# mj-will/aspire

Measured on AMD Instinct MI355X. Metric: particle-steps/sec (N x n_steps), 1M particles d=32; log-evidence err vs ref, higher is better.
Workload: dtype f64

## Files before the change

aspire_amd/csrc/asmc_common.h:

```cpp
#pragma once
#include <hip/hip_runtime.h>
#include <stdint.h>
#include <stdio.h>
#include <string.h>

#include "../../include/asmc.h"

#define ASMC_WAVE 64
#define ASMC_BLOCK 256
#define ASMC_MAX_BLOCKS 2048
#define ASMC_SCAN_TILE 2048
#define ASMC_PCN_MAX_GRID (1 << 20)
#define ASMC_GAMMA_BATCH 8
#define ASMC_MAX_PCN_STEPS 2048
#define BM_SC_N 256
#define BM_LG_N 128
#define BM_TAB_N (BM_SC_N + BM_LG_N)

void asmc_set_error(const char* fmt, ...);
void asmc_bm_table_host(double* tab);
struct asmc_ctx;
int asmc_count_nonfinite_enqueue(asmc_ctx* ctx, int64_t n, const double* v, hipStream_t st);
unsigned long long* asmc_count_slot(asmc_ctx* ctx);
struct asmc_ctx;
void asmc_prof_begin(asmc_ctx* ctx, const char* label, const void* kernel, hipStream_t st);
void asmc_poison_lds(asmc_ctx* ctx, hipStream_t st);
void asmc_prof_end(asmc_ctx* ctx, hipStream_t st);
#define ASMC_PROF_MAX 8192
#define ASMC_PROF_VARIANTS 256
#define ASMC_FIRST_ARG_(a, ...) a
#define ASMC_LAUNCH(ctx, st, label, ...)   \
    do {                                   \
        (ctx)->rec_n = 0;  \
        (ctx)->cs_n = 0;   \
        if ((ctx)->poison_lds) asmc_poison_lds((ctx), (st)); \
        asmc_prof_begin((ctx), (label), reinterpret_cast<const void*>(ASMC_FIRST_ARG_(__VA_ARGS__, 0)), (st)); \
        hipLaunchKernelGGL(__VA_ARGS__);   \
        asmc_prof_end((ctx), (st));        \
    } while (0)

#define ASMC_HIP(call)                                                                      \
    do {                                                                                    \
        hipError_t _e = (call);                                                             \
        if (_e != hipSuccess) {                                                             \
            asmc_set_error("%s failed: %s (%s:%d)", #call, hipGetErrorString(_e), __FILE__, \
                           __LINE__);                                                       \
            return ASMC_ERR_HIP;                                                            \
        }                                                                                   \
    } while (0)

// ... 38 lines not shown
    double* d_rec;
    const void* rec_src[3];
    int64_t rec_n;
    unsigned count_gen;
    uint64_t rec_token;
    const void* rec_hold_src[3];
    int64_t rec_hold_n;
    uint64_t rec_hold_token;
    const void* cs_x;
    int64_t cs_n;
    int cs_d, cs_grid;
    void* d_ysoa;
    void* d_xpad;
    size_t xpad_bytes;
    int d_max_pad;
    double* d_student;
    double* h_student;
    size_t ysoa_bytes;
    long long* d_counts;
    double* d_rho;
    unsigned long long* d_stretch;
    unsigned long long* d_mh;
    unsigned int* d_tilectr;
    unsigned int* d_bar;
    unsigned int bar_base[17];
    unsigned long long flow_nonfinite;
    int poison_lds;
    int isw_disabled;
    unsigned long long* d_pcgtab;
    long long* d_select;
    unsigned long long ptab_tag, ysplit_seq;
    double* d_ptab;
    double* d_bmtab;
    double* d_mmtab;
    double* d_f16tab;
    size_t f16tab_bytes;
    int (*count_hook)(void*, asmc_stream);
    void* count_hook_user;
    long long* count_cell;
    int count_cells;
    int64_t count_n_global;
    int mutate_defer, mutate_pending_steps;
    hipEvent_t ev_mutate;
    hipEvent_t ev_is;
    int is_result_pending;
    unsigned long long lq_nan;
    void* rccl_allreduce;
    void* rccl_comm;
    void* rccl_allgather;
    double* shard_st;
    int64_t n_tiles_max;
    int gram_blocks;
    size_t gram_cap;
    unsigned long long pcg_inc[2];
    int pcg_tab_valid;
    int prof_on;
    int prof_n;
    hipEvent_t* prof_ev;
    const char** prof_label;
    int prof_nv;
    const void* prof_vfn[ASMC_PROF_VARIANTS];
    long long prof_vcnt[ASMC_PROF_VARIANTS];
    double* h_pinned;
    unsigned ref_status_gen;
    double* h_gram;
    double* d_ref;
// ... 65 lines not shown
```

aspire_amd/csrc/asmc_ctx.hip:

```cpp
#include <dlfcn.h>
#include <stdarg.h>

#include <math.h>

#include "asmc_common.h"

static thread_local char g_err[512] = "";

void asmc_set_error(const char* fmt, ...) {
    va_list ap;
    va_start(ap, fmt);
    vsnprintf(g_err, sizeof(g_err), fmt, ap);
    va_end(ap);
}

__global__ __launch_bounds__(256) void k_poison_lds(int words) {
    extern __shared__ unsigned int s_poison[];
    for (int i = threadIdx.x; i < words; i += 256) s_poison[i] = 0xFFFFFFFFu;
    __syncthreads();
    if (s_poison[(threadIdx.x * 977) % words] != 0xFFFFFFFFu) __builtin_trap();
}
void asmc_poison_lds(asmc_ctx* ctx, hipStream_t st) {
    const int bytes = 160 * 1024 - 1024;
    static bool attr_set_dev[ASMC_MAX_DEVICES] = {false}; bool& attr_set = attr_set_dev[asmc_dev_slot(ctx)];
// ... 151 lines not shown
        if (e == hipSuccess) e = hipMalloc(p, bytes);
    };
    dmalloc((void**)&c->d_partials, sizeof(double) * ASMC_MAX_BLOCKS * ASMC_MAX_BETAS * 2);
    dmalloc((void**)&c->d_small, sizeof(double) * 4096);
    dmalloc((void**)&c->d_keys, sizeof(unsigned long long) * (ASMC_MAX_BETAS + 8));
    dmalloc((void**)&c->d_tiles, sizeof(double) * (size_t)(c->n_tiles_max * 4 + 64));
    dmalloc((void**)&c->d_tiles_i, sizeof(long long) * (size_t)(c->n_tiles_max * 8 + 64));
    c->gram_cap = (size_t)c->gram_blocks * d_max * d_max;
    if (c->gram_cap < (size_t)2048 * 1024) c->gram_cap = (size_t)2048 * 1024;
    dmalloc((void**)&c->d_gram, sizeof(double) * c->gram_cap);
    c->d_mmtab = nullptr;
    c->poison_lds = getenv("ASMC_POISON_LDS") != nullptr;
    c->d_max_pad = d_max <= 4 ? 4 : d_max <= 8 ? 8 : d_max <= 16 ? 16 : d_max <= 32 ? 32 : d_max <= 64 ? 64 : d_max <= 128 ? 128 : 0;
    dmalloc((void**)&c->d_mmtab, sizeof(double) * 2 * 144 * 64);
    dmalloc((void**)&c->d_guide, sizeof(unsigned int) * ((size_t)n_max + 8));
    dmalloc((void**)&c->d_tilectr, ASMC_TILECTR_BYTES + (size_t)n_max + 64);
    c->d_flags = c->d_tilectr ? reinterpret_cast<unsigned char*>(c->d_tilectr) + ASMC_TILECTR_BYTES : nullptr;
    dmalloc((void**)&c->d_gamma, sizeof(double) * ((size_t)ASMC_GAMMA_BATCH * (size_t)n_max + 64 * ASMC_GAMMA_BATCH));
    dmalloc((void**)&c->d_rec, sizeof(double) * 4 * (size_t)n_max);
    const size_t student = (size_t)d_max * (d_max + 1) + (size_t)(ASMC_STUDENT_MAX_ROWS / 64) * (d_max + 2);
    dmalloc((void**)&c->d_student, sizeof(double) * student);
    if (e == hipSuccess) e = hipHostMalloc((void**)&c->h_student, sizeof(double) * student, hipHostMallocDefault);
    dmalloc((void**)&c->d_counts, sizeof(long long) * (size_t)(ASMC_MAX_PCN_STEPS + ASMC_MAX_BLOCKS + n_max / 64 + 8));
    dmalloc((void**)&c->d_rho, sizeof(double) * (ASMC_MAX_PCN_STEPS + 8));
    dmalloc((void**)&c->d_stretch, sizeof(unsigned long long) * ASMC_MAX_PCN_STEPS);
    dmalloc((void**)&c->d_mh, sizeof(unsigned long long) * ASMC_MAX_PCN_STEPS);
    if (e == hipSuccess) e = hipMemset(c->d_tilectr, 0, ASMC_TILECTR_BYTES);
    dmalloc((void**)&c->d_bar, sizeof(unsigned int) * 1024 * 17);
    if (e == hipSuccess) e = hipMemset(c->d_bar, 0, sizeof(unsigned int) * 1024 * 17);
    dmalloc((void**)&c->d_pcgtab, sizeof(unsigned long long) * (64 * 4 + 8));
    dmalloc((void**)&c->d_select, sizeof(long long) * (2 * (ASMC_SELECT_THREADS / 64) + 8));
    dmalloc((void**)&c->d_ptab, sizeof(double) * (2 * 32 * 32 + 32 + 3 * ASMC_MAX_COMPONENTS * (1 + 2 * 32) + 64));
    dmalloc((void**)&c->d_bmtab, sizeof(double) * 2 * BM_TAB_N);
    dmalloc((void**)&c->d_ref, sizeof(double) * (128 + 128 * 128));
    if (e == hipSuccess) {
        double tab[2 * BM_TAB_N];
        asmc_bm_table_host(tab);
        e = hipMemcpy(c->d_bmtab, tab, sizeof(tab), hipMemcpyHostToDevice);
    }
    if (e == hipSuccess) e = hipHostMalloc((void**)&c->h_pinned, sizeof(double) * 8192, hipHostMallocDefault);
    if (e == hipSuccess) e = hipHostMalloc((void**)&c->h_gram, sizeof(double) * (128 + 128 * 128), hipHostMallocDefault);
    if (e != hipSuccess) {
        asmc_set_error("asmc_ctx_create: allocation failed: %s", hipGetErrorString(e));
        asmc_ctx_destroy(c);
        return ASMC_ERR_NOMEM;
    }
    *ctx_out = c;
    return ASMC_OK;
}

int asmc_ctx_destroy(asmc_ctx* c) {
    if (!c) return ASMC_OK;
    (void)hipSetDevice(c->device);
    (void)hipFree(c->d_partials);
    (void)hipFree(c->d_small);
    (void)hipFree(c->d_keys);
    (void)hipFree(c->d_tiles);
    (void)hipFree(c->d_tiles_i);
    (void)hipFree(c->d_gram);
    if (c->d_mmtab) (void)hipFree(c->d_mmtab);
    if (c->d_f16tab) (void)hipFree(c->d_f16tab);
    (void)hipFree(c->d_guide);
    (void)hipFree(c->d_gamma);
    (void)hipFree(c->d_student);
    if (c->h_student) (void)hipHostFree(c->h_student);
    if (c->d_ysoa) (void)hipFree(c->d_ysoa);
    if (c->d_xpad) (void)hipFree(c->d_xpad);
    (void)hipFree(c->d_counts);
    (void)hipFree(c->d_rho);
    (void)hipFree(c->d_stretch);
    (void)hipFree(c->d_mh);
    (void)hipFree(c->d_tilectr);
    (void)hipFree(c->d_rec);
    (void)hipFree(c->d_bar);
    (void)hipFree(c->d_pcgtab);
    (void)hipFree(c->d_select);
    (void)hipFree(c->d_ptab);
    (void)hipFree(c->d_bmtab);
    (void)hipFree(c->d_ref);
    if (c->prof_ev) {
        for (int i = 0; i < 2 * ASMC_PROF_MAX; i++) (void)hipEventDestroy(c->prof_ev[i]);
        delete[] c->prof_ev;
        delete[] c->prof_label;
    }
    if (c->h_pinned) (void)hipHostFree(c->h_pinned);
    if (c->h_gram) (void)hipHostFree(c->h_gram);
    if (c->ev_mutate) (void)hipEventDestroy(c->ev_mutate);
    if (c->ev_is) (void)hipEventDestroy(c->ev_is);
    delete c;
    return ASMC_OK;
}

}
```

aspire_amd/csrc/asmc_flow_dev.h:

```cpp
#pragma once
#include "asmc_common.h"

typedef float floatx16 __attribute__((ext_vector_type(16)));


__device__ __forceinline__ float flow_standardise(float x, float loc, float scale, float rcp) {
    const float a = x - loc;
    const float q0 = a * rcp;
    const float r = fmaf(-scale, q0, a);
    return fmaf(r, rcp, q0);
}

typedef float flow_std2 __attribute__((ext_vector_type(2)));
__device__ __forceinline__ flow_std2 flow_standardise2(flow_std2 x, flow_std2 loc, flow_std2 scale, flow_std2 rcp) {
    const flow_std2 a = x - loc;
    const flow_std2 q0 = a * rcp;
    const flow_std2 r = __builtin_elementwise_fma(-scale, q0, a);
    return __builtin_elementwise_fma(r, rcp, q0);
}

template <bool INVERSE>
__device__ __forceinline__ void flow_affine(float& x, float sraw, float t, float& ladj, int form) {
    if (form == 0) {
        const float sv = 2.0f - 4.0f * __builtin_amdgcn_rcpf(__expf(sraw) + 1.0f);
// ... 579 lines not shown
            if (overlap) {
#pragma unroll
                for (int c = 0; c < 4; c++)
                    if (c * NM / 4 == m) cvt(g + 1, c, c == 3);
            }
            __builtin_amdgcn_sched_barrier(0);
        }
        if (more) {
            if (!overlap) {
#pragma unroll
                for (int c = 0; c < 4; c++) cvt(g + 1, c, c == 3);
            }
            bh = pack(hp), bl = pack(lq);
            if (PREFETCH) {
#pragma unroll
                for (int nb = 0; nb < NBM; nb++) ah[nb] = ahn[nb], al[nb] = aln[nb];
            } else {
                a_load(g + 1, ah, al);
            }
            __builtin_amdgcn_sched_barrier(0);
        }
    }
    flow_f2 lacc = {0.0f, 0.0f};
#pragma unroll
    for (int q = 0; q < H / 2; q += 2)
        flow_affine2<false>(trans[q], trans[q + 1], o[q / 16][q % 16], o[(q + 1) / 16][(q + 1) % 16], o[(H / 2 + q) / 16][(H / 2 + q) % 16],
                            o[(H / 2 + q + 1) / 16][(H / 2 + q + 1) % 16], lacc, FORM >= 0 ? FORM : form);
    ladj += lacc.x + lacc.y;
}

template <int H, int W, int THREADS>
__device__ __forceinline__ void flow_stage_hs(float* __restrict__ sp, const float* __restrict__ packed, int n_layers) {
    using FD = FlowDims<H, W>;
    constexpr int L4 = FD::LAYER / 4, B4 = FD::BIAS / 4;
    const int total4 = n_layers * L4;
    for (int i4 = threadIdx.x; i4 < total4; i4 += THREADS) {
        const int in_layer = i4 % L4;
        if (in_layer < B4) {
            reinterpret_cast<float4*>(sp)[i4] = reinterpret_cast<const float4*>(packed)[i4];
            continue;
        }
        const int local = in_layer - B4;
        if ((local / 64) & 1) continue;
        const float4 f0 = reinterpret_cast<const float4*>(packed)[i4], f1 = reinterpret_cast<const float4*>(packed)[i4 + 64];
        const float xv[8] = {f0.x, f0.y, f0.z, f0.w, f1.x, f1.y, f1.z, f1.w};
        half8 hi, lo;
        float wmax = 0.0f;
        split8_f16<false>(xv, hi, lo, wmax);
        reinterpret_cast<half8*>(sp)[i4] = hi;
        reinterpret_cast<half8*>(sp)[i4 + 64] = lo;
    }
}
```

aspire_amd/csrc/asmc_pcn.hip:

```cpp
#include <stdlib.h>

#include <chrono>

#include "asmc_common.h"
#include "asmc_tile.h"
#include "asmc_pcn_dev.h"
#include "asmc_transform_dev.h"

template <typename T>
__device__ __forceinline__ double mixture_eval(const MixDev& m, int d, const char* row) {
    double best = -INFINITY;
    double terms[ASMC_MAX_COMPONENTS];
    const int C = m.C;
    for (int c = 0; c < C; c++) {
        double q = 0.0;
        const double* mu = m.mu + (size_t)c * d;
        const double* pr = m.prec + (size_t)c * d;
        for (int j = 0; j < d; j++) {
            const double t = row_get<T>(row, j) - mu[j];
            q = fma(t * t, pr[j], q);
        }
        const double v = m.logw[c] - 0.5 * q;
        terms[c] = v;
        best = fmax(best, v);
// ... 2911 lines not shown
        ASMC_LAUNCH_CHECK();
    }
    if (reg_ok) {
        pd.beta = prm->beta;
        pd.ll = to_dev(prm->log_likelihood);
        pd.lp = to_dev(prm->log_prior);
        pd.lq = pd.lp;
        pd.noise = prm->noise;
        ASMC_REQUIRE(pd.noise == ASMC_NOISE_F64 || pd.noise == ASMC_NOISE_F32, "bad noise mode");
        rc = pack_pcn_tables(ctx, pd, st, d_rho, *rho_inout_host);
        if (rc) return rc;
        long long* d_block = ctx->d_counts + ASMC_MAX_PCN_STEPS;
        int grid = 0;
        const bool soa = pcn_ensure_ysoa(ctx, n, d, prm->x_dtype, pd, st, asmc_pcn_flow_fused_ok(prm, flow));
        auto convert = [&](int mode) -> int {
            PcnDev pc = pd;
            pc.mode = !soa ? mode : mode == PCN_WHITEN ? PCN_WHITEN_S : PCN_UNWHITEN_XS;
            pc.noise = ASMC_NOISE_F64;
            if (prm->x_dtype == ASMC_F64)
                return launch_pcn_step<double, 0>(ctx, n, (double*)x, ll, lp, lq, pc, d_rho, 0, d_block, &grid, nullptr, nullptr, nullptr, st);
            return launch_pcn_step<float, 0>(ctx, n, (float*)x, ll, lp, lq, pc, d_rho, 0, d_block, &grid, nullptr, nullptr, nullptr, st);
        };
        rc = convert(PCN_WHITEN);
        if (rc) return rc;
        const bool fused = soa && asmc_pcn_flow_fused_ok(prm, flow);
        if (d_noise > 0 && !fused) {
            asmc_set_error("asmc_pcn_mutate_flow: the zero-padded form needs the one-kernel step");
            return ASMC_ERR_UNSUPPORTED;
        }
        if (fused) {
            ASMC_HIP(hipMemsetAsync(ctx->d_tilectr, 0, ASMC_TILECTR_BYTES + ((size_t)((n + 63) / 64) + 15) / 16 * 16, st));
            pd.tile_par = ctx->d_flags;
        }
        for (int t = 0; t < (fused ? n_steps : 0); t++) {
            const uint32_t step = step0 + (uint32_t)t;
            rc = pcn_prepare_gamma(ctx, n, pd, step, st);
            if (rc) return rc;
            PcnAdaptArgs ad = {ctx->d_tilectr + ASMC_MAX_PCN_STEPS + t,
                               reinterpret_cast<unsigned long long*>(ctx->d_tilectr + 2 * ASMC_MAX_PCN_STEPS),
                               ctx->count_hook ? ctx->count_cell : nullptr,
                               ctx->count_hook && t > 0 ? ctx->count_cell : nullptr, d_counts, d_rho, d_rho_hist,
                               prm->target_accept, ctx->count_hook ? ctx->count_n_global : n, t, prm->adapt, t == n_steps - 1};
            const int lag = prm->adapt >= 2 ? prm->adapt : 1;
            if (ctx->count_hook && lag > ctx->count_cells) {
                asmc_set_error("adapt_lag %d needs %d exchange cells, the installed hook has %d (asmc_pcn_set_count_cells)", lag, lag, ctx->count_cells);
                return ASMC_ERR_ARG;
            }
            rc = asmc_pcn_flow_fused_launch(ctx, n, prm->x_dtype == ASMC_F64 ? ASMC_F64 : ASMC_F32, ll, lp, lq, pd, flow, d_rho, step,
                                            ctx->d_tilectr + t, d_block, &grid, ad, st);
            if (rc) return rc;
            if (ctx->count_hook && ((t + 1) % lag == 0 || t == n_steps - 1)) {
                const int hrc = ctx->count_hook(ctx->count_hook_user, reinterpret_cast<asmc_stream>(st));
                if (hrc != 0) {
                    asmc_set_error("accept-count exchange hook failed (%d)", hrc);
                    return ASMC_ERR_ARG;
                }
                if (t == n_steps - 1) {
                    ASMC_LAUNCH(ctx, st, "k_pcn_adapt", k_pcn_adapt, dim3(1), dim3(1024), 0, st, 1,
                                (const long long*)ctx->count_cell, ctx->count_n_global, t, d_counts, d_rho, d_rho_hist,
                                prm->target_accept, prm->adapt, (const double*)(d_rho_hist + t), 1,
                                lag > 1 ? (const long long*)ctx->count_cell : (const long long*)nullptr);
                    ASMC_LAUNCH_CHECK();
                }
            }
        }
        for (int t = 0; t < (fused ? 0 : n_steps); t++) {
            const uint32_t step = step0 + (uint32_t)t;
            rc = pcn_prepare_gamma(ctx, n, pd, step, st);
            if (rc) return rc;
#define FLOW_STEP(TT, MD)                                                                                               \
    dispatch_pcn_reg_flow<TT, MD>(ctx, n, (TT*)x, (TT*)x_prop, ll, lp, lq, ll_new, lp_new, lq_new, pd, d_rho, step, d_block, \
                                  &grid, st)
            if (prm->x_dtype == ASMC_F64)
                rc = soa ? FLOW_STEP(double, PCN_FLOW_PROPOSE_S) : FLOW_STEP(double, PCN_FLOW_PROPOSE);
            else
                rc = soa ? FLOW_STEP(float, PCN_FLOW_PROPOSE_S) : FLOW_STEP(float, PCN_FLOW_PROPOSE);
            if (rc) return rc;
            rc = asmc_coupling_logprob(ctx, n, prm->x_dtype, x_prop, flow, lq_new, stream);
            if (rc) return rc;
            if (prm->x_dtype == ASMC_F64)
                rc = soa ? FLOW_STEP(double, PCN_FLOW_ACCEPT_S) : FLOW_STEP(double, PCN_FLOW_ACCEPT);
            else
// ... 309 lines not shown
```

aspire_amd/csrc/asmc_pcn_dev.h:

```cpp
#pragma once
#include "asmc_common.h"

bool asmc_flow_math_split();

struct PcnAdaptArgs {
    unsigned int* done;
    unsigned long long* nonfinite;
    long long* cell;
    const long long* prev_cell;
    long long* counts_out;
    double* rho;
    double* rho_hist;
    double target;
    int64_t n;
    int t, adapt;
    int last;
};

__device__ __forceinline__ double pcn_adapt_rho(double rho, long long c, int64_t n, double target, int t) {
    const double acc = (double)c / (double)n;
    double r = exp(log(rho) + (acc - target) / pow((double)(t + 1), 0.75));
    r = r < 1e-4 ? 1e-4 : r;
    r = r > 0.99 ? 0.99 : r;
    return r;
// ... 328 lines not shown
    int d_real;
    unsigned long long seed, gid0;
    int c_ll, c_lp, c_lq;
    const double* bmtab;
    unsigned char* tile_par;
    int d_noise;
};


template <typename T>
__device__ __forceinline__ double soa_load(__amdgpu_buffer_rsrc_t r, unsigned voff, unsigned soff) {
    if constexpr (sizeof(T) == 8) {
        const auto v = __builtin_amdgcn_raw_buffer_load_b64(r, (int)voff, (int)soff, 0);
        return __builtin_bit_cast(double, v);
    } else {
        const unsigned v = __builtin_amdgcn_raw_buffer_load_b32(r, (int)voff, (int)soff, 0);
        return (double)__uint_as_float(v);
    }
}
template <typename T>
__device__ __forceinline__ void soa_store(__amdgpu_buffer_rsrc_t r, unsigned voff, unsigned soff, double x) {
    if constexpr (sizeof(T) == 8) {
        using u2 = decltype(__builtin_amdgcn_raw_buffer_load_b64(r, 0, 0, 0));
        __builtin_amdgcn_raw_buffer_store_b64(__builtin_bit_cast(u2, x), r, (int)voff, (int)soff, 0);
    } else {
        __builtin_amdgcn_raw_buffer_store_b32(__float_as_uint((float)x), r, (int)voff, (int)soff, 0);
    }
}


bool asmc_pcn_flow_fused_ok(const asmc_pcn_params* prm, const asmc_coupling* f);
int asmc_pcn_flow_fused_launch(asmc_ctx* ctx, int64_t n, int x_dtype, double* ll, double* lp, double* lq, const PcnDev& pd,
                               const asmc_coupling* f, const double* rho_ptr, uint32_t step, unsigned int* tile_counter,
                               long long* block_counts, int* grid_out, const PcnAdaptArgs& adapt, hipStream_t st);

#define MM_WHITEN 0
#define MM_STEP 1
#define MM_UNWHITEN 2
#define MM_STEP_T 3
#define MM_XPROPOSE 4
#define MM_XPROPOSE_T 5
#define MM_UNWHITEN_X 6
bool asmc_pcn_mm_supported(int d, const void* x);
int asmc_pcn_mm_pack(asmc_ctx* ctx, const PcnDev& pd, hipStream_t st);
int asmc_pcn_flow16_tables(asmc_ctx* ctx, const PcnDev& pd, const asmc_coupling* f, hipStream_t st);
int asmc_pcn_flow16_launch(asmc_ctx* ctx, int64_t n, int x_dtype, void* x, double* ll, double* lp, double* lq, const PcnDev& pd,
                           const asmc_coupling* f, const double* rho_ptr, uint32_t step, long long* block_counts, int* grid_out,
                           unsigned long long* nonfinite, hipStream_t st);
int asmc_pcn_mm_launch(asmc_ctx* ctx, int64_t n, int x_dtype, void* x, double* ll, double* lp, double* lq, const PcnDev& pd,
                       int mode, const double* rho_ptr, uint32_t step, long long* block_counts, int* grid_out,
                       hipStream_t st);
bool asmc_gram_mm_supported(int d, const void* x);
int asmc_gram_mm_launch(asmc_ctx* ctx, int64_t n, int d, int x_dtype, const void* x, const double* d_center, int* grid_out,
                        hipStream_t st, double* out2, double n_div);
```

aspire_amd/csrc/asmc_pcn_fused.hip:

```cpp
#include <stdlib.h>

#include "asmc_common.h"
#include <type_traits>
#include "asmc_pcn_dev.h"
#include "asmc_flow_dev.h"

#ifndef FUSED_THREADS
#define FUSED_THREADS 512
#endif

#define FUSED_TL_DOUBLES 1368
#define FUSED_MAX_COMPONENTS 4
#ifndef MV_DEPTH
#define MV_DEPTH 4
#endif
typedef double double2v __attribute__((ext_vector_type(2)));
__host__ __device__ constexpr int mv_group(int bi) {
    int g = 0;
    while ((g + 1) * (g + 2) <= bi) g++;
    return g;
}
template <int I, int N, typename F>
__device__ __forceinline__ void mv_for_each(F& f) {
    if constexpr (I < N) {
        f(std::integral_constant<int, I>{});
        mv_for_each<I + 1, N>(f);
    }
}
#ifndef FUSED_INPLACE
#define FUSED_INPLACE 1
#endif
#ifndef FUSED_MVMFMA
#define FUSED_MVMFMA FUSED_INPLACE
#endif
typedef double fused_d4 __attribute__((ext_vector_type(4)));
__device__ __forceinline__ void fused_swap32(double& x, double& y) {
    const unsigned long long xb = __builtin_bit_cast(unsigned long long, x), yb = __builtin_bit_cast(unsigned long long, y);
    const auto lo = __builtin_amdgcn_permlane32_swap((unsigned)xb, (unsigned)yb, false, false);
    const auto hi = __builtin_amdgcn_permlane32_swap((unsigned)(xb >> 32), (unsigned)(yb >> 32), false, false);
    x = __builtin_bit_cast(double, ((unsigned long long)hi[0] << 32) | lo[0]);
    y = __builtin_bit_cast(double, ((unsigned long long)hi[1] << 32) | lo[1]);
}
__device__ __forceinline__ void fused_swap16(double& x, double& y) {
    const unsigned long long xb = __builtin_bit_cast(unsigned long long, x), yb = __builtin_bit_cast(unsigned long long, y);
    const auto lo = __builtin_amdgcn_permlane16_swap((unsigned)xb, (unsigned)yb, false, false);
    const auto hi = __builtin_amdgcn_permlane16_swap((unsigned)(xb >> 32), (unsigned)(yb >> 32), false, false);
    x = __builtin_bit_cast(double, ((unsigned long long)hi[0] << 32) | lo[0]);
    y = __builtin_bit_cast(double, ((unsigned long long)hi[1] << 32) | lo[1]);
}
__device__ __forceinline__ void fused_transpose4(double& q0, double& q1, double& q2, double& q3) {
    fused_swap32(q0, q2);
    fused_swap32(q1, q3);
    fused_swap16(q0, q1);
    fused_swap16(q2, q3);
}
#ifndef HS1P_PREFETCH
#define HS1P_PREFETCH false
#endif
#ifndef FUSED_PRIO_A
#define FUSED_PRIO_A 2
#define FUSED_PRIO_B 1
#endif
#ifndef MV_CHUNK
#define MV_CHUNK 8
#endif
template <typename T, int W, int NOISE, bool HS, int KIND = ASMC_FLOW_COUPLING, bool MIX = false>
__global__ __launch_bounds__(FUSED_THREADS) void k_pcn_flow_fused(
    int64_t n, double* __restrict__ ll, double* __restrict__ lp, double* __restrict__ lq, const double* __restrict__ ptab,
    PcnScalars p, const double* rho_ptr, uint32_t step, const float* __restrict__ packed, int n_layers,
    const float* __restrict__ loc, const float* __restrict__ scale, float ladj0, float base_const,
    unsigned int* __restrict__ tile_counter, long long* __restrict__ block_counts, PcnAdaptArgs ad, int par_words, int affine) {
    constexpr int D = 32, H = 16, THREADS = FUSED_THREADS;
    constexpr int HF = KIND == ASMC_FLOW_MAF ? 32 : H;
    static_assert(KIND == ASMC_FLOW_COUPLING || HS, "the autoregressive variant runs the split-fp16 layers only");
    using FD = FlowDims<HF, W>;
    extern __shared__ __align__(16) float sp[];
    if (HS) {
        flow_stage_hs<HF, W, THREADS>(sp, packed, n_layers);
    } else {
        const int total4 = n_layers * FD::LAYER / 4;
        for (int base = 0; base < total4; base += THREADS * 8) {
            float4 tmp[8];
#pragma unroll
            for (int q = 0; q < 8; q++) {
                const int i4 = base + q * THREADS + threadIdx.x;
                tmp[q] = i4 < total4 ? reinterpret_cast<const float4*>(packed)[i4] : make_float4(0.f, 0.f, 0.f, 0.f);
            }
#pragma unroll
            for (int q = 0; q < 8; q++) {
                const int i4 = base + q * THREADS + threadIdx.x;
                if (i4 < total4) reinterpret_cast<float4*>(sp)[i4] = tmp[q];
            }
        }
    }
    double* tl = reinterpret_cast<double*>(sp + (size_t)n_layers * FD::LAYER);
    constexpr int T_MU = D * D, T_LLMU = T_MU + D, T_LLPR = T_LLMU + D, T_LPMU = T_LLPR + D, T_LPPR = T_LPMU + D,
                  T_LOGW = T_LPPR + D, T_LOC = T_LOGW + 2;
    static_assert(T_LOC + 3 * D / 2 <= FUSED_TL_DOUBLES, "pCN tables");
    constexpr int M_MU = 12 * 64, M_MIX = M_MU + D, M_LOGW = M_MIX + 2 * FUSED_MAX_COMPONENTS * 2 * D, M_LOC = M_LOGW + 2 * FUSED_MAX_COMPONENTS;
    static_assert(M_LOC + 3 * D / 2 <= FUSED_TL_DOUBLES, "pCN tables (matrix-core variant)");
    constexpr bool MVM = FUSED_MVMFMA && FUSED_INPLACE;
    {
        const double* m0g = ptab + 2 * PTAB_TRI(D) + D;
        const int dr = (p.d_noise > 0 && p.d_noise < D) ? p.d_noise : D;
        const int dhalf = KIND == ASMC_FLOW_MAF ? 16 : dr / 2;
        auto nat = [&](int r) -> int {
            const int c = r < 16 ? (r < dhalf ? r : -1) : (r - 16 + dhalf);
            return (c >= 0 && c < dr) ? c : -1;
        };
        if (MVM) {
            for (int e = threadIdx.x; e < 12 * 64; e += THREADS) {
                const int slot = e >> 6, l = e & 63, mb = slot < 4 ? 0 : 1, sidx = slot < 4 ? slot : slot - 4;
                const int i = l & 15, j = nat(16 * mb + 4 * (i & 3) + (i >> 2)), k = 4 * sidx + (l >> 4);
                tl[e] = (j >= 0 && k <= j) ? ptab[j * (j + 1) / 2 + k] : 0.0;
            }
            for (int e = threadIdx.x; e < D; e += THREADS) {
                const int j = nat(16 * ((e >> 2) & 1) + 4 * (e >> 3) + (e & 3));
                tl[M_MU + e] = j >= 0 ? ptab[2 * PTAB_TRI(D) + j] : 0.0;
                reinterpret_cast<float*>(tl + M_LOC)[e] = j >= 0 ? loc[j] : 0.0f;
                reinterpret_cast<float*>(tl + M_LOC)[D + e] = j >= 0 ? scale[j] : 1.0f;
                reinterpret_cast<float*>(tl + M_LOC)[2 * D + e] = j >= 0 ? 1.0f / scale[j] : 1.0f;
            }
            for (int e = threadIdx.x; e < 2 * FUSED_MAX_COMPONENTS * D; e += THREADS) {
                const int tc = e / D, er = e % D, tt = tc / FUSED_MAX_COMPONENTS, c = tc % FUSED_MAX_COMPONENTS;
                const int j = nat(16 * ((er >> 2) & 1) + 4 * (er >> 3) + (er & 3));
                const bool live = j >= 0 && c < (tt == 0 ? p.c_ll : p.c_lp);
                const double* mg = m0g + (size_t)tt * PTAB_MIX(D);
                tl[M_MIX + tc * 2 * D + er] = live ? mg[ASMC_MAX_COMPONENTS + c * D + j] : 0.0;
                tl[M_MIX + tc * 2 * D + D + er] = live ? mg[ASMC_MAX_COMPONENTS * (1 + D) + c * D + j] : 0.0;
            }
            if (threadIdx.x < 2 * FUSED_MAX_COMPONENTS) {
                const int tt = threadIdx.x / FUSED_MAX_COMPONENTS, c = threadIdx.x % FUSED_MAX_COMPONENTS;
                tl[M_LOGW + threadIdx.x] = c < (tt == 0 ? p.c_ll : p.c_lp) ? m0g[(size_t)tt * PTAB_MIX(D) + c] : -INFINITY;
            }
        } else {
            for (int e = threadIdx.x; e < D * D; e += THREADS) {
                const int j = e / D, k = e - j * D;
                tl[e] = k <= j ? ptab[j * (j + 1) / 2 + k] : 0.0;
            }
            for (int e = threadIdx.x; e < D; e += THREADS) {
                tl[T_MU + e] = ptab[2 * PTAB_TRI(D) + e];
                tl[T_LLMU + e] = m0g[ASMC_MAX_COMPONENTS + e];
                tl[T_LLPR + e] = m0g[ASMC_MAX_COMPONENTS * (1 + D) + e];
                tl[T_LPMU + e] = m0g[PTAB_MIX(D) + ASMC_MAX_COMPONENTS + e];
                tl[T_LPPR + e] = m0g[PTAB_MIX(D) + ASMC_MAX_COMPONENTS * (1 + D) + e];
                reinterpret_cast<float*>(tl + T_LOC)[e] = loc[e];
                reinterpret_cast<float*>(tl + T_LOC)[D + e] = scale[e];
                reinterpret_cast<float*>(tl + T_LOC)[2 * D + e] = 1.0f / scale[e];
            }
        }
        if (!MVM && threadIdx.x == 0) tl[T_LOGW] = m0g[0], tl[T_LOGW + 1] = m0g[PTAB_MIX(D)];
    }
    bm_d2* bmt = reinterpret_cast<bm_d2*>(tl + FUSED_TL_DOUBLES);
    if (NOISE == ASMC_NOISE_F64) bm_tab_stage<THREADS>(bmt, p.bmtab);
    unsigned* const par_bits = reinterpret_cast<unsigned*>(bmt + BM_TAB_N);
    for (int wd = threadIdx.x; wd < par_words; wd += THREADS) {
        const uint4 b0 = reinterpret_cast<const uint4*>(p.tile_par)[2 * wd], b1 = reinterpret_cast<const uint4*>(p.tile_par)[2 * wd + 1];
        const unsigned q[8] = {b0.x, b0.y, b0.z, b0.w, b1.x, b1.y, b1.z, b1.w};
        unsigned bits = 0;
#pragma unroll
        for (int k = 0; k < 8; k++) {
            const unsigned nib = (((q[k] & 0x01010101u) * 0x01020408u) >> 24) & 0xFu;
            bits |= nib << (4 * k);
        }
        par_bits[wd] = bits;
    }
    __syncthreads();
    const int lane = threadIdx.x & 63, wave = threadIdx.x >> 6, hh = lane >> 5;
    const bool first_on_simd = __builtin_amdgcn_readfirstlane(wave) < 4;
#ifdef FUSED_STAGGER
    if (!first_on_simd) {
#pragma unroll 1
        for (int i = 0; i < FUSED_STAGGER; i++) __builtin_amdgcn_s_sleep(127);
    }
#endif
    double rho;
    if (ad.prev_cell) {
        const double rp = ad.rho_hist[ad.t - 1];
        if (ad.adapt <= 1) {
            const long long cp = *ad.prev_cell;
            rho = ad.adapt ? pcn_adapt_rho(rp, cp, ad.n, ad.target, ad.t - 1) : rp;
            if (blockIdx.x == 0 && threadIdx.x == 0) ad.counts_out[ad.t - 1] = cp;
        } else if (ad.t % ad.adapt == 0) {
            double r = rp;
            for (int tp = ad.t - ad.adapt; tp < ad.t; tp++) {
                const long long ct = ad.prev_cell[tp % ad.adapt];
                r = pcn_adapt_rho(r, ct, ad.n, ad.target, tp);
                if (blockIdx.x == 0 && threadIdx.x == 0) ad.counts_out[tp] = ct;
            }
            rho = r;
        } else {
            rho = rp;
        }
    } else {
        rho = *rho_ptr;
    }
    if (ad.cell && blockIdx.x == 0 && threadIdx.x == 0) ad.rho_hist[ad.t] = rho;
    const double a = sqrt(1.0 - rho * rho);
// ... 609 lines not shown
        const unsigned int tk = __hip_atomic_fetch_add(ad.done, 1u, __ATOMIC_RELAXED, __HIP_MEMORY_SCOPE_AGENT);
        s_last = (tk == gridDim.x - 1u);
        if (s_last) __builtin_amdgcn_fence(__ATOMIC_ACQUIRE, "agent");
    }
    __syncthreads();
    if (!s_last) return;
    long long c = 0;
    for (int b = threadIdx.x; b < (int)gridDim.x; b += THREADS)
        c += __hip_atomic_load(&block_counts[b], __ATOMIC_RELAXED, __HIP_MEMORY_SCOPE_AGENT);
    c = wave_sum_ll(c);
    __syncthreads();
    if (lane == 0) s_cnt[wave] = c;
    __syncthreads();
    if (threadIdx.x == 0) {
        c = 0;
        for (int w = 0; w < THREADS / 64; w++) c += s_cnt[w];
        if (ad.cell) {
            ad.cell[ad.adapt >= 2 ? ad.t % ad.adapt : 0] = c;
            return;
        }
        ad.counts_out[ad.t] = c;
        ad.rho_hist[ad.t] = rho;
        if (ad.adapt == 1) {
            *ad.rho = pcn_adapt_rho(rho, c, ad.n, ad.target, ad.t);
        } else if (ad.adapt >= 2 && ((ad.t + 1) % ad.adapt == 0 || ad.last)) {
            double r = rho;
            for (int tp = ad.t - (ad.t % ad.adapt); tp <= ad.t; tp++)
                r = pcn_adapt_rho(r, tp == ad.t ? c : ad.counts_out[tp], ad.n, ad.target, tp);
            *ad.rho = r;
        }
    }
}

template <typename T>
static int launch_pcn_flow_fused(asmc_ctx* ctx, int64_t n, double* ll, double* lp, double* lq, const PcnDev& pd,
                                 const asmc_coupling* f, const double* rho_ptr, uint32_t step, unsigned int* tile_counter,
                                 long long* block_counts, int* grid_out, const PcnAdaptArgs& adapt, hipStream_t st) {
    PcnScalars ps;
    ps.beta = pd.beta;
    ps.nu = pd.nu;
    ps.gam = pd.gam;
    ps.ys = pd.ys;
    ps.n_pad = pd.n_pad;
    ps.d_real = pd.d;
    ps.d_noise = pd.d_noise;
    ps.seed = pd.seed;
    ps.gid0 = pd.gid0;
    ps.c_ll = pd.ll.C;
    ps.c_lp = pd.lp.C;
    ps.c_lq = 0;
    ps.bmtab = pd.bmtab;
    ps.tile_par = pd.tile_par;
    const float ladj0 = (float)(-f->log_scale_sum);
    const float base_const = (float)(-0.5 * f->dims * 1.8378770664093453);
    const int64_t n_tiles = (n + 63) / 64;
    const int grid = (int)(n_tiles < (int64_t)ctx->num_cu * (FUSED_THREADS / 64) ? (n_tiles + FUSED_THREADS / 64 - 1) / (FUSED_THREADS / 64) : ctx->num_cu);
    *grid_out = grid;
    const bool hs = asmc_flow_math_split();
    const bool mix = pd.ll.C > 1 || pd.lp.C > 1;
#define ASMC_FUSED_CASE_K(WW, NZ, HSV, KD) ASMC_FUSED_CASE_KM(WW, NZ, HSV, KD, false)
#define ASMC_FUSED_CASE_KM(WW, NZ, HSV, KD, MX)                                                                           \
    if (f->hidden == WW && pd.noise == NZ && hs == HSV && f->kind == KD && mix == MX) {                                   \
        auto kern = k_pcn_flow_fused<T, WW, NZ, HSV, KD, MX>;                                                                 \
        const size_t lds0 = (size_t)f->n_layers * FlowDims<(KD == ASMC_FLOW_MAF ? 32 : 16), WW>::LAYER * sizeof(float) + FUSED_TL_DOUBLES * sizeof(double) + BM_TAB_N * sizeof(bm_d2); \
        const size_t par_bytes = (size_t)((n_tiles + 31) / 32) * 4;    \
        const int par_words = (!FUSED_INPLACE && lds0 + par_bytes <= 160 * 1024) ? (int)(par_bytes / 4) : 0;                     \
        const size_t lds = lds0 + (size_t)par_words * 4;                                                                     \
        static size_t attr_lds_dev[ASMC_MAX_DEVICES] = {0}; size_t& attr_lds = attr_lds_dev[asmc_dev_slot(ctx)];                                                                                      \
        if (lds > 64 * 1024 && lds > attr_lds) {                                                                         \
            ASMC_HIP(hipFuncSetAttribute(reinterpret_cast<const void*>(kern), hipFuncAttributeMaxDynamicSharedMemorySize, (int)lds)); \
            attr_lds = lds;                                                                                              \
        }                                                                                                                \
        ASMC_LAUNCH(ctx, st, "k_pcn_flow_fused", kern, dim3(grid), dim3(FUSED_THREADS), lds, st, n, ll, lp, lq,                     \
                    (const double*)ctx->d_ptab, ps, rho_ptr, step, f->packed_dev, (int)f->n_layers, f->loc_dev, f->scale_dev, \
                    ladj0, base_const, tile_counter, block_counts, adapt, par_words, KD == ASMC_FLOW_MAF ? (int)f->affine : 0);  \
        ASMC_LAUNCH_CHECK();                                                                                             \
        return ASMC_OK;                                                                                                  \
    }
#define ASMC_FUSED_CASE(WW, NZ, HSV) ASMC_FUSED_CASE_K(WW, NZ, HSV, ASMC_FLOW_COUPLING)
    ASMC_FUSED_CASE(64, ASMC_NOISE_F64, true)
#ifndef FUSED_ONLY_HEADLINE
    ASMC_FUSED_CASE_KM(64, ASMC_NOISE_F64, true, ASMC_FLOW_COUPLING, true)
    ASMC_FUSED_CASE_KM(64, ASMC_NOISE_F32, true, ASMC_FLOW_COUPLING, true)
    ASMC_FUSED_CASE(64, ASMC_NOISE_F64, false)
    ASMC_FUSED_CASE(64, ASMC_NOISE_F32, true)
    ASMC_FUSED_CASE(64, ASMC_NOISE_F32, false)
    ASMC_FUSED_CASE(32, ASMC_NOISE_F64, true)
    ASMC_FUSED_CASE(32, ASMC_NOISE_F64, false)
    ASMC_FUSED_CASE(32, ASMC_NOISE_F32, true)
    ASMC_FUSED_CASE(32, ASMC_NOISE_F32, false)
    ASMC_FUSED_CASE(128, ASMC_NOISE_F64, true)
    ASMC_FUSED_CASE(128, ASMC_NOISE_F64, false)
    ASMC_FUSED_CASE(128, ASMC_NOISE_F32, true)
    ASMC_FUSED_CASE(128, ASMC_NOISE_F32, false)
    ASMC_FUSED_CASE_K(64, ASMC_NOISE_F64, true, ASMC_FLOW_MAF)
    ASMC_FUSED_CASE_K(64, ASMC_NOISE_F32, true, ASMC_FLOW_MAF)
    ASMC_FUSED_CASE_K(32, ASMC_NOISE_F64, true, ASMC_FLOW_MAF)
    ASMC_FUSED_CASE_K(32, ASMC_NOISE_F32, true, ASMC_FLOW_MAF)
#endif
#undef ASMC_FUSED_CASE
#undef ASMC_FUSED_CASE_K
#undef ASMC_FUSED_CASE_KM
    asmc_set_error("fused flow step: unsupported flow (kind %d, hidden width %d)", (int)f->kind, (int)f->hidden);
    return ASMC_ERR_UNSUPPORTED;
}

bool asmc_pcn_flow_fused_ok(const asmc_pcn_params* prm, const asmc_coupling* f) {
    if (getenv("ASMC_FLOW_SPLIT")) return false;
    if (prm->d != 32 || f->dims > 32 || f->dims < 2) return false;
    if (f->dims != 32 && !(FUSED_MVMFMA && FUSED_INPLACE)) return false;
    if (f->kind == ASMC_FLOW_COUPLING && (f->dims % 2)) return false;
    const bool mvm = FUSED_MVMFMA && FUSED_INPLACE && f->kind == ASMC_FLOW_COUPLING && f->hidden == 64 && asmc_flow_math_split();
    const int cmax = mvm ? FUSED_MAX_COMPONENTS : 1;
    if (prm->log_likelihood.n_components < 1 || prm->log_likelihood.n_components > cmax) return false;
    if (prm->log_prior.n_components < 1 || prm->log_prior.n_components > cmax) return false;
    if (!(f->hidden == 32 || f->hidden == 64 || f->hidden == 128)) return false;
    if (f->kind == ASMC_FLOW_MAF) {
        if (!asmc_flow_math_split() || f->hidden == 128) return false;
        const size_t per_tr = (size_t)((2 * (f->hidden / 32) + 2) * 32 + f->hidden * 32 + f->hidden * f->hidden + 2 * 32 * f->hidden) * sizeof(float);
        return per_tr * (size_t)f->n_layers + FUSED_TL_DOUBLES * sizeof(double) + BM_TAB_N * sizeof(bm_d2) <= 160 * 1024;
    }
    const size_t per_layer = (size_t)((2 * (f->hidden / 32) + 1) * 32 + f->hidden * 16 + f->hidden * f->hidden + 2 * 16 * f->hidden) * sizeof(float);
    return per_layer * (size_t)f->n_layers + FUSED_TL_DOUBLES * sizeof(double) + BM_TAB_N * sizeof(bm_d2) <= 160 * 1024;
}


int asmc_pcn_flow_fused_launch(asmc_ctx* ctx, int64_t n, int x_dtype, double* ll, double* lp, double* lq, const PcnDev& pd,
                               const asmc_coupling* f, const double* rho_ptr, uint32_t step, unsigned int* tile_counter,
                               long long* block_counts, int* grid_out, const PcnAdaptArgs& adapt, hipStream_t st) {
    if (x_dtype == ASMC_F64)
        return launch_pcn_flow_fused<double>(ctx, n, ll, lp, lq, pd, f, rho_ptr, step, tile_counter, block_counts, grid_out, adapt, st);
    return launch_pcn_flow_fused<float>(ctx, n, ll, lp, lq, pd, f, rho_ptr, step, tile_counter, block_counts, grid_out, adapt, st);
}
```

Baseline: 3.495 billion.

## Prebuild fused-kernel LDS image once per sweep and bulk-copy it per block

Adds a one-block staging kernel that builds the fused pCN step's LDS contents once per call: split-fp16 flow weights, pCN tables and the Box-Muller table, written to a device buffer. Each block of the per-step fused kernel then loads this image with wide coalesced reads held in registers and stores it to LDS, instead of recomputing the fp16 splits and tables itself. The inline staging loop is also batched so more global loads are in flight at once. The aim is to cut per-block prologue cost, at the price of many extra registers per thread to hold the image (up to 160 KB split over the block) and one extra launch per sweep. An environment variable can restore inline staging.

After: 3.553 billion (median of 6 runs). 1.7% higher.

```diff
diff --git a/aspire_amd/csrc/asmc_common.h b/aspire_amd/csrc/asmc_common.h
--- a/aspire_amd/csrc/asmc_common.h
+++ b/aspire_amd/csrc/asmc_common.h
@@ -16,6 +16,7 @@
 #define BM_SC_N 256
 #define BM_LG_N 128
 #define BM_TAB_N (BM_SC_N + BM_LG_N)
+#define ASMC_FUSED_IMAGE_BYTES (160 * 1024)
 
 void asmc_set_error(const char* fmt, ...);
 void asmc_bm_table_host(double* tab);
@@ -120,6 +121,7 @@
     unsigned long long ptab_tag, ysplit_seq;
     double* d_ptab;
     double* d_bmtab;
+    void* d_fimg;
     double* d_mmtab;
     double* d_f16tab;
     size_t f16tab_bytes;
diff --git a/aspire_amd/csrc/asmc_ctx.hip b/aspire_amd/csrc/asmc_ctx.hip
--- a/aspire_amd/csrc/asmc_ctx.hip
+++ b/aspire_amd/csrc/asmc_ctx.hip
@@ -207,6 +207,7 @@
     dmalloc((void**)&c->d_select, sizeof(long long) * (2 * (ASMC_SELECT_THREADS / 64) + 8));
     dmalloc((void**)&c->d_ptab, sizeof(double) * (2 * 32 * 32 + 32 + 3 * ASMC_MAX_COMPONENTS * (1 + 2 * 32) + 64));
     dmalloc((void**)&c->d_bmtab, sizeof(double) * 2 * BM_TAB_N);
+    dmalloc((void**)&c->d_fimg, ASMC_FUSED_IMAGE_BYTES);
     dmalloc((void**)&c->d_ref, sizeof(double) * (128 + 128 * 128));
     if (e == hipSuccess) {
         double tab[2 * BM_TAB_N];
@@ -252,6 +253,7 @@
     (void)hipFree(c->d_select);
     (void)hipFree(c->d_ptab);
     (void)hipFree(c->d_bmtab);
+    (void)hipFree(c->d_fimg);
     (void)hipFree(c->d_ref);
     if (c->prof_ev) {
         for (int i = 0; i < 2 * ASMC_PROF_MAX; i++) (void)hipEventDestroy(c->prof_ev[i]);
diff --git a/aspire_amd/csrc/asmc_flow_dev.h b/aspire_amd/csrc/asmc_flow_dev.h
--- a/aspire_amd/csrc/asmc_flow_dev.h
+++ b/aspire_amd/csrc/asmc_flow_dev.h
@@ -635,22 +635,35 @@
 template <int H, int W, int THREADS>
 __device__ __forceinline__ void flow_stage_hs(float* __restrict__ sp, const float* __restrict__ packed, int n_layers) {
     using FD = FlowDims<H, W>;
-    constexpr int L4 = FD::LAYER / 4, B4 = FD::BIAS / 4;
+    constexpr int L4 = FD::LAYER / 4, B4 = FD::BIAS / 4, BATCH = 8;
     const int total4 = n_layers * L4;
-    for (int i4 = threadIdx.x; i4 < total4; i4 += THREADS) {
-        const int in_layer = i4 % L4;
-        if (in_layer < B4) {
-            reinterpret_cast<float4*>(sp)[i4] = reinterpret_cast<const float4*>(packed)[i4];
-            continue;
-        }
-        const int local = in_layer - B4;
-        if ((local / 64) & 1) continue;
-        const float4 f0 = reinterpret_cast<const float4*>(packed)[i4], f1 = reinterpret_cast<const float4*>(packed)[i4 + 64];
-        const float xv[8] = {f0.x, f0.y, f0.z, f0.w, f1.x, f1.y, f1.z, f1.w};
-        half8 hi, lo;
-        float wmax = 0.0f;
-        split8_f16<false>(xv, hi, lo, wmax);
-        reinterpret_cast<half8*>(sp)[i4] = hi;
-        reinterpret_cast<half8*>(sp)[i4 + 64] = lo;
-    }
-}
+    const float4* __restrict__ g4 = reinterpret_cast<const float4*>(packed);
+    for (int base = threadIdx.x; base < total4; base += THREADS * BATCH) {
+        float4 f0[BATCH], f1[BATCH];
+#pragma unroll
+        for (int q = 0; q < BATCH; q++) {
+            const int i4 = base + q * THREADS, in_layer = i4 % L4;
+            const bool in = i4 < total4, bias = in_layer < B4;
+            const bool pair = in && !bias && !(((in_layer - B4) / 64) & 1);
+            f0[q] = f1[q] = make_float4(0.f, 0.f, 0.f, 0.f);
+            if ((in && bias) || pair) f0[q] = g4[i4];
+            if (pair) f1[q] = g4[i4 + 64];
+        }
+#pragma unroll
+        for (int q = 0; q < BATCH; q++) {
+            const int i4 = base + q * THREADS, in_layer = i4 % L4;
+            if (i4 >= total4) continue;
+            if (in_layer < B4) {
+                reinterpret_cast<float4*>(sp)[i4] = f0[q];
+                continue;
+            }
+            if (((in_layer - B4) / 64) & 1) continue;
+            const float xv[8] = {f0[q].x, f0[q].y, f0[q].z, f0[q].w, f1[q].x, f1[q].y, f1[q].z, f1[q].w};
+            half8 hi, lo;
+            float wmax = 0.0f;
+            split8_f16<false>(xv, hi, lo, wmax);
+            reinterpret_cast<half8*>(sp)[i4] = hi;
+            reinterpret_cast<half8*>(sp)[i4 + 64] = lo;
+        }
+    }
+}
diff --git a/aspire_amd/csrc/asmc_pcn.hip b/aspire_amd/csrc/asmc_pcn.hip
--- a/aspire_amd/csrc/asmc_pcn.hip
+++ b/aspire_amd/csrc/asmc_pcn.hip
@@ -2967,6 +2967,11 @@
             ASMC_HIP(hipMemsetAsync(ctx->d_tilectr, 0, ASMC_TILECTR_BYTES + ((size_t)((n + 63) / 64) + 15) / 16 * 16, st));
             pd.tile_par = ctx->d_flags;
         }
+        int img_words = 0;
+        if (fused) {
+            rc = asmc_pcn_flow_fused_stage(ctx, pd, flow, &img_words, st);
+            if (rc) return rc;
+        }
         for (int t = 0; t < (fused ? n_steps : 0); t++) {
             const uint32_t step = step0 + (uint32_t)t;
             rc = pcn_prepare_gamma(ctx, n, pd, step, st);
@@ -2982,7 +2987,7 @@
                 return ASMC_ERR_ARG;
             }
             rc = asmc_pcn_flow_fused_launch(ctx, n, prm->x_dtype == ASMC_F64 ? ASMC_F64 : ASMC_F32, ll, lp, lq, pd, flow, d_rho, step,
-                                            ctx->d_tilectr + t, d_block, &grid, ad, st);
+                                            ctx->d_tilectr + t, d_block, &grid, ad, img_words, st);
             if (rc) return rc;
             if (ctx->count_hook && ((t + 1) % lag == 0 || t == n_steps - 1)) {
                 const int hrc = ctx->count_hook(ctx->count_hook_user, reinterpret_cast<asmc_stream>(st));
diff --git a/aspire_amd/csrc/asmc_pcn_dev.h b/aspire_amd/csrc/asmc_pcn_dev.h
--- a/aspire_amd/csrc/asmc_pcn_dev.h
+++ b/aspire_amd/csrc/asmc_pcn_dev.h
@@ -384,7 +384,8 @@
 bool asmc_pcn_flow_fused_ok(const asmc_pcn_params* prm, const asmc_coupling* f);
 int asmc_pcn_flow_fused_launch(asmc_ctx* ctx, int64_t n, int x_dtype, double* ll, double* lp, double* lq, const PcnDev& pd,
                                const asmc_coupling* f, const double* rho_ptr, uint32_t step, unsigned int* tile_counter,
-                               long long* block_counts, int* grid_out, const PcnAdaptArgs& adapt, hipStream_t st);
+                               long long* block_counts, int* grid_out, const PcnAdaptArgs& adapt, int img_words, hipStream_t st);
+int asmc_pcn_flow_fused_stage(asmc_ctx* ctx, const PcnDev& pd, const asmc_coupling* f, int* words_out, hipStream_t st);
 
 #define MM_WHITEN 0
 #define MM_STEP 1
diff --git a/aspire_amd/csrc/asmc_pcn_fused.hip b/aspire_amd/csrc/asmc_pcn_fused.hip
--- a/aspire_amd/csrc/asmc_pcn_fused.hip
+++ b/aspire_amd/csrc/asmc_pcn_fused.hip
@@ -34,6 +34,7 @@
 #define FUSED_MVMFMA FUSED_INPLACE
 #endif
 typedef double fused_d4 __attribute__((ext_vector_type(4)));
+typedef unsigned fused_u4 __attribute__((ext_vector_type(4)));
 __device__ __forceinline__ void fused_swap32(double& x, double& y) {
     const unsigned long long xb = __builtin_bit_cast(unsigned long long, x), yb = __builtin_bit_cast(unsigned long long, y);
     const auto lo = __builtin_amdgcn_permlane32_swap((unsigned)xb, (unsigned)yb, false, false);
@@ -64,17 +65,20 @@
 #ifndef MV_CHUNK
 #define MV_CHUNK 8
 #endif
-template <typename T, int W, int NOISE, bool HS, int KIND = ASMC_FLOW_COUPLING, bool MIX = false>
-__global__ __launch_bounds__(FUSED_THREADS) void k_pcn_flow_fused(
-    int64_t n, double* __restrict__ ll, double* __restrict__ lp, double* __restrict__ lq, const double* __restrict__ ptab,
-    PcnScalars p, const double* rho_ptr, uint32_t step, const float* __restrict__ packed, int n_layers,
-    const float* __restrict__ loc, const float* __restrict__ scale, float ladj0, float base_const,
-    unsigned int* __restrict__ tile_counter, long long* __restrict__ block_counts, PcnAdaptArgs ad, int par_words, int affine) {
-    constexpr int D = 32, H = 16, THREADS = FUSED_THREADS;
-    constexpr int HF = KIND == ASMC_FLOW_MAF ? 32 : H;
-    static_assert(KIND == ASMC_FLOW_COUPLING || HS, "the autoregressive variant runs the split-fp16 layers only");
+constexpr int FUSED_D = 32;
+constexpr int T_MU = FUSED_D * FUSED_D, T_LLMU = T_MU + FUSED_D, T_LLPR = T_LLMU + FUSED_D, T_LPMU = T_LLPR + FUSED_D, T_LPPR = T_LPMU + FUSED_D,
+              T_LOGW = T_LPPR + FUSED_D, T_LOC = T_LOGW + 2;
+static_assert(T_LOC + 3 * FUSED_D / 2 <= FUSED_TL_DOUBLES, "pCN tables");
+constexpr int M_MU = 12 * 64, M_MIX = M_MU + FUSED_D, M_LOGW = M_MIX + 2 * FUSED_MAX_COMPONENTS * 2 * FUSED_D, M_LOC = M_LOGW + 2 * FUSED_MAX_COMPONENTS;
+static_assert(M_LOC + 3 * FUSED_D / 2 <= FUSED_TL_DOUBLES, "pCN tables (matrix-core variant)");
+constexpr bool MVM = FUSED_MVMFMA && FUSED_INPLACE;
+
+template <int W, int NOISE, bool HS, int KIND>
+__device__ __forceinline__ void fused_stage_tables(float* __restrict__ sp, const double* __restrict__ ptab, const PcnScalars& p,
+                                                   const float* __restrict__ packed, int n_layers, const float* __restrict__ loc,
+                                                   const float* __restrict__ scale) {
+    constexpr int D = FUSED_D, THREADS = FUSED_THREADS, HF = KIND == ASMC_FLOW_MAF ? 32 : 16;
     using FD = FlowDims<HF, W>;
-    extern __shared__ __align__(16) float sp[];
     if (HS) {
         flow_stage_hs<HF, W, THREADS>(sp, packed, n_layers);
     } else {
@@ -94,12 +98,6 @@
         }
     }
     double* tl = reinterpret_cast<double*>(sp + (size_t)n_layers * FD::LAYER);
-    constexpr int T_MU = D * D, T_LLMU = T_MU + D, T_LLPR = T_LLMU + D, T_LPMU = T_LLPR + D, T_LPPR = T_LPMU + D,
-                  T_LOGW = T_LPPR + D, T_LOC = T_LOGW + 2;
-    static_assert(T_LOC + 3 * D / 2 <= FUSED_TL_DOUBLES, "pCN tables");
-    constexpr int M_MU = 12 * 64, M_MIX = M_MU + D, M_LOGW = M_MIX + 2 * FUSED_MAX_COMPONENTS * 2 * D, M_LOC = M_LOGW + 2 * FUSED_MAX_COMPONENTS;
-    static_assert(M_LOC + 3 * D / 2 <= FUSED_TL_DOUBLES, "pCN tables (matrix-core variant)");
-    constexpr bool MVM = FUSED_MVMFMA && FUSED_INPLACE;
     {
         const double* m0g = ptab + 2 * PTAB_TRI(D) + D;
         const int dr = (p.d_noise > 0 && p.d_noise < D) ? p.d_noise : D;
@@ -151,8 +149,48 @@
         }
         if (!MVM && threadIdx.x == 0) tl[T_LOGW] = m0g[0], tl[T_LOGW + 1] = m0g[PTAB_MIX(D)];
     }
+    if (NOISE == ASMC_NOISE_F64) bm_tab_stage<THREADS>(reinterpret_cast<bm_d2*>(tl + FUSED_TL_DOUBLES), p.bmtab);
+}
+template <int W, int NOISE, int KIND>
+__host__ __device__ constexpr int fused_image_words(int n_layers) {
+    return (int)(((size_t)n_layers * FlowDims<(KIND == ASMC_FLOW_MAF ? 32 : 16), W>::LAYER * sizeof(float) + FUSED_TL_DOUBLES * sizeof(double) +
+                  (NOISE == ASMC_NOISE_F64 ? BM_TAB_N * sizeof(bm_d2) : 0)) / 16);
+}
+template <int W, int NOISE, bool HS, int KIND>
+__global__ __launch_bounds__(FUSED_THREADS) void k_fused_stage_image(const double* __restrict__ ptab, PcnScalars p, const float* __restrict__ packed,
+                                                                     int n_layers, const float* __restrict__ loc, const float* __restrict__ scale,
+                                                                     fused_u4* __restrict__ img, int img_words) {
+    extern __shared__ __align__(16) float sp[];
+    fused_stage_tables<W, NOISE, HS, KIND>(sp, ptab, p, packed, n_layers, loc, scale);
+    __syncthreads();
+    for (int i = threadIdx.x; i < img_words; i += FUSED_THREADS) img[i] = reinterpret_cast<const fused_u4*>(sp)[i];
+}
+
+template <typename T, int W, int NOISE, bool HS, int KIND = ASMC_FLOW_COUPLING, bool MIX = false>
+__global__ __launch_bounds__(FUSED_THREADS) void k_pcn_flow_fused(
+    int64_t n, double* __restrict__ ll, double* __restrict__ lp, double* __restrict__ lq, const double* __restrict__ ptab,
+    PcnScalars p, const double* rho_ptr, uint32_t step, const float* __restrict__ packed, int n_layers,
+    const float* __restrict__ loc, const float* __restrict__ scale, float ladj0, float base_const,
+    unsigned int* __restrict__ tile_counter, long long* __restrict__ block_counts, PcnAdaptArgs ad, int par_words, int affine,
+    const fused_u4* __restrict__ img, int img_words) {
+    constexpr int D = FUSED_D, H = 16, THREADS = FUSED_THREADS;
+    constexpr int HF = KIND == ASMC_FLOW_MAF ? 32 : H;
+    static_assert(KIND == ASMC_FLOW_COUPLING || HS, "the autoregressive variant runs the split-fp16 layers only");
+    using FD = FlowDims<HF, W>;
+    extern __shared__ __align__(16) float sp[];
+    constexpr int IMG_Q = ASMC_FUSED_IMAGE_BYTES / 16 / THREADS;
+    fused_u4 iw[IMG_Q];
+    if (img != nullptr) {
+#pragma unroll
+        for (int q = 0; q < IMG_Q; q++) {
+            const int i4 = q * THREADS + (int)threadIdx.x;
+            iw[q] = img[i4 < img_words ? i4 : img_words - 1];
+        }
+    } else {
+        fused_stage_tables<W, NOISE, HS, KIND>(sp, ptab, p, packed, n_layers, loc, scale);
+    }
+    double* tl = reinterpret_cast<double*>(sp + (size_t)n_layers * FD::LAYER);
     bm_d2* bmt = reinterpret_cast<bm_d2*>(tl + FUSED_TL_DOUBLES);
-    if (NOISE == ASMC_NOISE_F64) bm_tab_stage<THREADS>(bmt, p.bmtab);
     unsigned* const par_bits = reinterpret_cast<unsigned*>(bmt + BM_TAB_N);
     for (int wd = threadIdx.x; wd < par_words; wd += THREADS) {
         const uint4 b0 = reinterpret_cast<const uint4*>(p.tile_par)[2 * wd], b1 = reinterpret_cast<const uint4*>(p.tile_par)[2 * wd + 1];
@@ -164,6 +202,14 @@
             bits |= nib << (4 * k);
         }
         par_bits[wd] = bits;
+    }
+    if (img != nullptr) {
+        __builtin_amdgcn_sched_barrier(0);
+#pragma unroll
+        for (int q = 0; q < IMG_Q; q++) {
+            const int i4 = q * THREADS + (int)threadIdx.x;
+            if (i4 < img_words) reinterpret_cast<fused_u4*>(sp)[i4] = iw[q];
+        }
     }
     __syncthreads();
     const int lane = threadIdx.x & 63, wave = threadIdx.x >> 6, hh = lane >> 5;
@@ -839,10 +885,7 @@
     }
 }
 
-template <typename T>
-static int launch_pcn_flow_fused(asmc_ctx* ctx, int64_t n, double* ll, double* lp, double* lq, const PcnDev& pd,
-                                 const asmc_coupling* f, const double* rho_ptr, uint32_t step, unsigned int* tile_counter,
-                                 long long* block_counts, int* grid_out, const PcnAdaptArgs& adapt, hipStream_t st) {
+static PcnScalars fused_scalars(const PcnDev& pd) {
     PcnScalars ps;
     ps.beta = pd.beta;
     ps.nu = pd.nu;
@@ -858,6 +901,15 @@
     ps.c_lq = 0;
     ps.bmtab = pd.bmtab;
     ps.tile_par = pd.tile_par;
+    return ps;
+}
+
+template <typename T>
+static int launch_pcn_flow_fused(asmc_ctx* ctx, int64_t n, double* ll, double* lp, double* lq, const PcnDev& pd,
+                                 const asmc_coupling* f, const double* rho_ptr, uint32_t step, unsigned int* tile_counter,
+                                 long long* block_counts, int* grid_out, const PcnAdaptArgs& adapt, int img_words, hipStream_t st) {
+    const PcnScalars ps = fused_scalars(pd);
+    const fused_u4* img = img_words > 0 ? reinterpret_cast<const fused_u4*>(ctx->d_fimg) : nullptr;
     const float ladj0 = (float)(-f->log_scale_sum);
     const float base_const = (float)(-0.5 * f->dims * 1.8378770664093453);
     const int64_t n_tiles = (n + 63) / 64;
@@ -880,7 +932,7 @@
         }                                                                                                                \
         ASMC_LAUNCH(ctx, st, "k_pcn_flow_fused", kern, dim3(grid), dim3(FUSED_THREADS), lds, st, n, ll, lp, lq,                     \
                     (const double*)ctx->d_ptab, ps, rho_ptr, step, f->packed_dev, (int)f->n_layers, f->loc_dev, f->scale_dev, \
-                    ladj0, base_const, tile_counter, block_counts, adapt, par_words, KD == ASMC_FLOW_MAF ? (int)f->affine : 0);  \
+                    ladj0, base_const, tile_counter, block_counts, adapt, par_words, KD == ASMC_FLOW_MAF ? (int)f->affine : 0, img, img_words);  \
         ASMC_LAUNCH_CHECK();                                                                                             \
         return ASMC_OK;                                                                                                  \
     }
@@ -932,10 +984,56 @@
 }
 
 
+int asmc_pcn_flow_fused_stage(asmc_ctx* ctx, const PcnDev& pd, const asmc_coupling* f, int* words_out, hipStream_t st) {
+    *words_out = 0;
+    const char* mode = getenv("ASMC_FUSED_STAGE");
+    if (mode && !strcmp(mode, "inline")) return ASMC_OK;
+    const PcnScalars ps = fused_scalars(pd);
+    const bool hs = asmc_flow_math_split();
+#define ASMC_STAGE_CASE(WW, NZ, HSV, KD)                                                                                 \
+    if (f->hidden == WW && pd.noise == NZ && hs == HSV && f->kind == KD) {                                               \
+        auto kern = k_fused_stage_image<WW, NZ, HSV, KD>;                                                                \
+        const int words = fused_image_words<WW, NZ, KD>((int)f->n_layers);                                               \
+        const size_t lds = (size_t)words * 16;                                                                           \
+        if (lds > ASMC_FUSED_IMAGE_BYTES) {                                                                              \
+            asmc_set_error("fused flow step: LDS image of %zu bytes", lds);                                              \
+            return ASMC_ERR_UNSUPPORTED;                                                                                 \
+        }                                                                                                                \
+        static size_t attr_lds_dev[ASMC_MAX_DEVICES] = {0}; size_t& attr_lds = attr_lds_dev[asmc_dev_slot(ctx)];         \
+        if (lds > 64 * 1024 && lds > attr_lds) {                                                                         \
+            ASMC_HIP(hipFuncSetAttribute(reinterpret_cast<const void*>(kern), hipFuncAttributeMaxDynamicSharedMemorySize, (int)lds)); \
+            attr_lds = lds;                                                                                              \
+        }                                                                                                                \
+        ASMC_LAUNCH(ctx, st, "k_fused_stage_image", kern, dim3(1), dim3(FUSED_THREADS), lds, st, (const double*)ctx->d_ptab, ps, \
+                    f->packed_dev, (int)f->n_layers, f->loc_dev, f->scale_dev, reinterpret_cast<fused_u4*>(ctx->d_fimg), words); \
+        ASMC_LAUNCH_CHECK();                                                                                             \
+        *words_out = words;                                                                                              \
+        return ASMC_OK;                                                                                                  \
+    }
+#define ASMC_STAGE_CASES(WW)                                   \
+    ASMC_STAGE_CASE(WW, ASMC_NOISE_F64, true, ASMC_FLOW_COUPLING)  \
+    ASMC_STAGE_CASE(WW, ASMC_NOISE_F32, true, ASMC_FLOW_COUPLING)  \
+    ASMC_STAGE_CASE(WW, ASMC_NOISE_F64, false, ASMC_FLOW_COUPLING) \
+    ASMC_STAGE_CASE(WW, ASMC_NOISE_F32, false, ASMC_FLOW_COUPLING)
+    ASMC_STAGE_CASES(64)
+#ifndef FUSED_ONLY_HEADLINE
+    ASMC_STAGE_CASES(32)
+    ASMC_STAGE_CASES(128)
+    ASMC_STAGE_CASE(64, ASMC_NOISE_F64, true, ASMC_FLOW_MAF)
+    ASMC_STAGE_CASE(64, ASMC_NOISE_F32, true, ASMC_FLOW_MAF)
+    ASMC_STAGE_CASE(32, ASMC_NOISE_F64, true, ASMC_FLOW_MAF)
+    ASMC_STAGE_CASE(32, ASMC_NOISE_F32, true, ASMC_FLOW_MAF)
+#endif
+#undef ASMC_STAGE_CASES
+#undef ASMC_STAGE_CASE
+    asmc_set_error("fused flow step: unsupported flow (kind %d, hidden width %d)", (int)f->kind, (int)f->hidden);
+    return ASMC_ERR_UNSUPPORTED;
+}
+
 int asmc_pcn_flow_fused_launch(asmc_ctx* ctx, int64_t n, int x_dtype, double* ll, double* lp, double* lq, const PcnDev& pd,
                                const asmc_coupling* f, const double* rho_ptr, uint32_t step, unsigned int* tile_counter,
-                               long long* block_counts, int* grid_out, const PcnAdaptArgs& adapt, hipStream_t st) {
+                               long long* block_counts, int* grid_out, const PcnAdaptArgs& adapt, int img_words, hipStream_t st) {
     if (x_dtype == ASMC_F64)
-        return launch_pcn_flow_fused<double>(ctx, n, ll, lp, lq, pd, f, rho_ptr, step, tile_counter, block_counts, grid_out, adapt, st);
-    return launch_pcn_flow_fused<float>(ctx, n, ll, lp, lq, pd, f, rho_ptr, step, tile_counter, block_counts, grid_out, adapt, st);
-}
+        return launch_pcn_flow_fused<double>(ctx, n, ll, lp, lq, pd, f, rho_ptr, step, tile_counter, block_counts, grid_out, adapt, img_words, st);
+    return launch_pcn_flow_fused<float>(ctx, n, ll, lp, lq, pd, f, rho_ptr, step, tile_counter, block_counts, grid_out, adapt, img_words, st);
+}
```
